# ushasigh/srsran-edgeric-5g

Measured on AMD Instinct MI355X. Metric: pdsch_slots_per_sec, higher is better.
Workload: dtype u32 bit-packed GF(2) + bf16 grid + f32 IQ

## Files before the change

### srsran-edgeric-5g_amd/csrc/bits_device.h

```cpp
#pragma once

#include "nrphy_internal.h"

namespace nrphy {

constexpr int WAVE = 64;

#ifdef NRPHY_WG_TRACE
constexpr uint32_t WG_TRACE_MAX = 16384;
__device__ uint64_t g_wg_trace[8 * WG_TRACE_MAX];
#define NRPHY_WG_TRACE_MARK(slot)                                              \
  do {                                                                         \
    if (threadIdx.x == 0 && blockIdx.x < WG_TRACE_MAX) {                       \
      g_wg_trace[8 * blockIdx.x + (slot)] = wall_clock64();                    \
    }                                                                          \
  } while (0)
#define NRPHY_WG_TRACE_WHERE(role)                                                                              \
  do {                                                                                                          \
    if (threadIdx.x == 0 && blockIdx.x < WG_TRACE_MAX) {                                                        \
      const uint64_t hw = (uint32_t)__builtin_amdgcn_s_getreg((31 << 11) | 4), xcc = (uint32_t)__builtin_amdgcn_s_getreg((31 << 11) | 20); \
      g_wg_trace[8 * blockIdx.x + 7] = ((uint64_t)(role) << 60) | ((xcc & 0xFu) << 32) | hw;                     \
    }                                                                                                           \
  } while (0)
#else
// ... 169 lines not shown
}

__device__ __forceinline__ uint32_t byte_masks_msb_first(uint32_t bits4)
{
  const uint32_t spread = ((bits4 >> 3) & 1u) | (((bits4 >> 2) & 1u) << 8) | (((bits4 >> 1) & 1u) << 16) | ((bits4 & 1u) << 24);
  return spread * 0xFFu;
}

__device__ __forceinline__ uint32_t negate_bytes(uint32_t x, uint32_t m)
{
  const uint32_t a = x ^ m, b = m & 0x01010101u;
  return ((a & 0x7F7F7F7Fu) + b) ^ (a & 0x80808080u);
}

__device__ __forceinline__ uint32_t gold_matvec(const uint32_t* rows, uint32_t state, uint32_t lane)
{
  uint32_t bit = (lane < 31u) ? (__popc(rows[lane & 31u] & state) & 1u) : 0u;
  return (uint32_t)__ballot(bit != 0) & 0x7FFFFFFFu;
}

__device__ __forceinline__ void wave_lds_fence()
{
  asm volatile("s_waitcnt lgkmcnt(0)" ::: "memory");
}

__device__ inline void gold_sequence_wave(const GoldTables* gold, const uint32_t* x1_words, uint32_t c_init,
                                          uint32_t nwords, uint32_t* __restrict__ out, uint32_t* scratch,
                                          uint32_t lane)
{
  uint32_t state = c_init & 0x7FFFFFFFu;
  state = gold_matvec(gold->x2_jump[6], state, lane);
  state = gold_matvec(gold->x2_jump[9], state, lane);
  state = gold_matvec(gold->x2_jump[10], state, lane);
  if (lane < 31u && lane < nwords) {
    uint32_t word = 0;
#pragma unroll 8
    for (uint32_t t = 0; t != 32; ++t) {
      word |= (__popc(gold->x2_head[t][lane] & state) & 1u) << (31u - t);
    }
    scratch[lane] = word;
  }
  wave_lds_fence();
  for (uint32_t base = 31; base < nwords; base += 28) {
    const uint32_t k = base + lane;
    if (lane < 28u && k < nwords) {
      scratch[k] = scratch[k - 28] ^ scratch[k - 29] ^ scratch[k - 30] ^ scratch[k - 31];
    }
    wave_lds_fence();
  }
  for (uint32_t k = lane; k < nwords; k += WAVE) {
    out[k] = scratch[k] ^ x1_words[k];
  }
}

#ifndef NRPHY_GOLD_LEVEL
#define NRPHY_GOLD_LEVEL 64
#endif
constexpr uint32_t GOLD_MAX_LEVEL  = NRPHY_GOLD_LEVEL;
constexpr uint32_t GOLD_RING_WORDS = 64 * GOLD_MAX_LEVEL;

__device__ __forceinline__ void lds_barrier()
{
  asm volatile("s_waitcnt lgkmcnt(0)\n\ts_barrier" ::: "memory");
}

template <uint32_t NT, bool WITH_X1 = true>
__device__ inline void gold_sequence_workgroup(const GoldTables* gold, const uint32_t* x1_words, uint32_t c_init,
                                               uint32_t first_word, uint32_t nwords, uint32_t* __restrict__ out,
                                               uint32_t* ring, uint32_t tid)
{
  constexpr uint32_t MASK = GOLD_RING_WORDS - 1;
  constexpr uint32_t PER  = (28u * GOLD_MAX_LEVEL + NT - 1u) / NT;
  const uint32_t     lane = tid & (WAVE - 1);
  if (nwords == 0) {
    return;
  }
  static_assert(NT == 4 * WAVE, "four waves share the seed words");
  if (tid < 31u) {
    ring[tid] = 0u;
  }
  if (tid < WAVE) {
    uint32_t       state  = c_init & 0x7FFFFFFFu;
    const uint32_t offset = 1600u + 32u * first_word;
    uint32_t row[GOLD_JUMP_BITS];
#pragma unroll
    for (uint32_t k = 0; k != GOLD_JUMP_BITS; ++k) {
      row[k] = ((offset >> k) & 1u) ? gold->x2_jump[k][lane & 31u] : 0u;
    }
#pragma unroll
    for (uint32_t k = 0; k != GOLD_JUMP_BITS; ++k) {
      if ((offset >> k) & 1u) {
        const uint32_t bit = (lane < 31u) ? (__popc(row[k] & state) & 1u) : 0u;
        state              = (uint32_t)__ballot(bit != 0) & 0x7FFFFFFFu;
      }
    }
    if (lane == 0) {
      ring[GOLD_RING_WORDS - 1u] = state;
    }
  }
  lds_barrier();
  {
    const uint32_t state = ring[GOLD_RING_WORDS - 1u];
    const uint32_t t0    = 8u * (tid / WAVE);
    if (lane < 31u) {
      uint32_t head[8];
#pragma unroll
      for (uint32_t t = 0; t != 8; ++t) {
        head[t] = gold->x2_head[t0 + t][lane];
      }
      uint32_t word = 0;
#pragma unroll
      for (uint32_t t = 0; t != 8; ++t) {
        word |= (__popc(head[t] & state) & 1u) << (31u - (t0 + t));
      }
      atomicOr(&ring[lane], word);
    }
  }
  lds_barrier();
  uint32_t pw[PER], px[PER];
  uint32_t pbeg = 0, pend = nwords < 31u ? nwords : 31u;
#pragma unroll
  for (uint32_t i = 0; i != PER; ++i) {
    const uint32_t k = tid + i * NT;
    pw[i]            = (k < pend) ? ring[k] : 0u;
    px[i]            = (WITH_X1 && k < pend) ? x1_words[first_word + k] : 0u;
  }
  uint32_t m = 1, have = 31;
  auto step = [&](uint32_t (&nw)[PER], uint32_t (&nx)[PER], const uint32_t (&ow)[PER], const uint32_t (&ox)[PER]) {
    while (m < GOLD_MAX_LEVEL && have >= 62u * m) {
      m *= 2u;
    }
    const uint32_t end = have + 28u * m < nwords ? have + 28u * m : nwords;
#pragma unroll
    for (uint32_t i = 0; i != PER; ++i) {
      const uint32_t k = have + tid + i * NT;
      nx[i]            = (WITH_X1 && k < end) ? x1_words[first_word + k] : 0u;
    }
#pragma unroll
    for (uint32_t i = 0; i != PER; ++i) {
      const uint32_t k = have + tid + i * NT;
      nw[i]            = 0;
      if (k < end) {
        nw[i] = ring[(k - 28u * m) & MASK] ^ ring[(k - 29u * m) & MASK] ^ ring[(k - 30u * m) & MASK] ^
                ring[(k - 31u * m) & MASK];
        ring[k & MASK] = nw[i];
      }
    }
#pragma unroll
    for (uint32_t i = 0; i != PER; ++i) {
      const uint32_t k = pbeg + tid + i * NT;
      if (k < pend) {
        out[k] = ow[i] ^ ox[i];
      }
    }
    pbeg = have;
    pend = end;
    lds_barrier();
    have = end;
  };
  uint32_t qw[PER], qx[PER];
  bool     in_q = false;
  while (have < nwords) {
    step(qw, qx, pw, px);
    in_q = true;
    if (have >= nwords) {
      break;
    }
    step(pw, px, qw, qx);
    in_q = false;
  }
#pragma unroll
  for (uint32_t i = 0; i != PER; ++i) {
    const uint32_t k = pbeg + tid + i * NT;
    if (k < pend) {
      out[k] = in_q ? (qw[i] ^ qx[i]) : (pw[i] ^ px[i]);
    }
  }
  lds_barrier();
}

constexpr uint32_t GOLD_SEED_ROWS  = 31;
constexpr uint32_t GOLD_SEED_WORDS = GOLD_SEED_ROWS * WAVE;

template <class OnBlock>
__device__ inline void gold_sequence_blocks_wave(const GoldTables* gold, uint32_t c_init, uint32_t first_word, uint32_t nwords,
                                                 uint32_t* area, uint32_t lane, OnBlock&& on_block)
{
  if (nwords == 0) {
    return;
  }
  uint32_t state = c_init & 0x7FFFFFFFu;
  {
    const uint32_t offset = 1600u + 32u * first_word;
    uint32_t       row[GOLD_JUMP_BITS];
#pragma unroll
    for (uint32_t k = 0; k != GOLD_JUMP_BITS; ++k) {
      row[k] = ((offset >> k) & 1u) ? gold->x2_jump[k][lane & 31u] : 0u;
    }
#pragma unroll
    for (uint32_t k = 0; k != GOLD_JUMP_BITS; ++k) {
      if ((offset >> k) & 1u) {
        const uint32_t bit = (lane < 31u) ? (__popc(row[k] & state) & 1u) : 0u;
        state              = (uint32_t)__ballot(bit != 0) & 0x7FFFFFFFu;
      }
    }
  }
  NRPHY_WG_TRACE_MARK(1);
  if (lane < 31u) {
    uint32_t head[32];
#pragma unroll
    for (uint32_t t = 0; t != 32; ++t) {
      head[t] = gold->x2_head[t][lane];
    }
    uint32_t word = 0;
#pragma unroll
    for (uint32_t t = 0; t != 32; ++t) {
      word |= (__popc(head[t] & state) & 1u) << (31u - t);
    }
    area[lane] = word;
  }
  wave_lds_fence();
  NRPHY_WG_TRACE_MARK(2);
  const uint32_t need = nwords < GOLD_SEED_WORDS ? nwords : GOLD_SEED_WORDS;
  for (uint32_t have = 31u, m = 1u; have < need;) {
    while (m < 32u && have >= 62u * m) {
      m *= 2u;
    }
    const uint32_t end = have + 28u * m < need ? have + 28u * m : need;
    for (uint32_t k = have + lane; k < end; k += WAVE) {
      area[k] = __builtin_amdgcn_bitop3_b32(area[k - 28u * m], area[k - 29u * m], area[k - 30u * m], 0x96) ^
                area[k - 31u * m];
    }
    wave_lds_fence();
    have = end;
  }
  NRPHY_WG_TRACE_MARK(3);
  on_block(0u, need);
  NRPHY_WG_TRACE_MARK(4);
  const uint32_t rows = (nwords + WAVE - 1u) / WAVE;
  if (rows <= GOLD_SEED_ROWS) {
    return;
  }
  uint32_t w[GOLD_SEED_ROWS];
#pragma unroll
  for (uint32_t i = 0; i != GOLD_SEED_ROWS; ++i) {
    w[i] = area[i * WAVE + lane];
  }
  for (uint32_t base = GOLD_SEED_ROWS; base < rows; base += GOLD_SEED_ROWS) {
#pragma unroll
    for (uint32_t i = 0; i != GOLD_SEED_ROWS; ++i) {
      w[i] ^= __builtin_amdgcn_bitop3_b32(w[(i + 1u) % GOLD_SEED_ROWS], w[(i + 2u) % GOLD_SEED_ROWS],
                                          w[(i + 3u) % GOLD_SEED_ROWS], 0x96);
      area[i * WAVE + lane] = w[i];
    }
    wave_lds_fence();
    const uint32_t left = nwords - base * WAVE;
    on_block(base * WAVE, left < GOLD_SEED_WORDS ? left : GOLD_SEED_WORDS);
  }
}

constexpr uint32_t GOLD_EXPAND_MAX_WORDS = 703;

template <uint32_t M>
__device__ __forceinline__ uint32_t gold_expand_step(uint32_t* x2, uint32_t have, uint32_t need, uint32_t lane)
{
  if (have >= need) {
    return have;
  }
  const uint32_t end = have + 28u * M < need ? have + 28u * M : need;
#pragma unroll
  for (uint32_t s = 0; s != (28u * M + WAVE - 1u) / WAVE; ++s) {
    if (have + WAVE * s >= end) {
      break;
    }
    const uint32_t k = have + lane + WAVE * s;
    if (k < end) {
      uint32_t* b = x2 + (k - 31u * M);
      b[31u * M]  = __builtin_amdgcn_bitop3_b32(b[3u * M], b[2u * M], b[M], 0x96) ^ b[0];
    }
  }
  wave_lds_fence();
  return end;
}

__device__ inline void gold_expand_seed_wave(uint32_t* x2, uint32_t seed_word, uint32_t need, uint32_t lane)
{
  if (lane < 31u) {
    x2[lane] = seed_word;
  }
  wave_lds_fence();
  uint32_t have = 31u;
  have = gold_expand_step<1>(x2, have, need, lane);
  have = gold_expand_step<1>(x2, have, need, lane);
  have = gold_expand_step<2>(x2, have, need, lane);
  have = gold_expand_step<4>(x2, have, need, lane);
  have = gold_expand_step<8>(x2, have, need, lane);
  have = gold_expand_step<8>(x2, have, need, lane);
}

constexpr int TB_CRC_THREADS = 256;

constexpr int TB_CRC_WPT = NRPHY_CRC_WORDS_PER_THREAD;
static_assert(TB_CRC_REGION_WORDS == TB_CRC_WPT * TB_CRC_THREADS, "words per thread");

__device__ __forceinline__ uint32_t crc_advance(const uint32_t* tab, uint32_t reg)
{
  return tab[reg & 0xFFu] ^ tab[256u + ((reg >> 8) & 0xFFu)] ^ tab[512u + ((reg >> 16) & 0xFFu)] ^ tab[768u + (reg >> 24)];
}

constexpr uint32_t TB_CRC_LDS_WORDS = 4 * 1024 + 2 * TB_CRC_THREADS;

__device__ inline uint32_t tbcrc_regions_workgroup(const TbCrcTables* tables, uint32_t sel, CrcPoly c, const uint32_t* tbw, uint32_t n,
                                                   uint32_t region0, uint32_t count, uint32_t factor, uint32_t* lds, uint32_t tid)
{
  uint32_t*       y32 = lds;
  uint32_t*       y1k = lds + 1024;
  uint32_t*       y8k = lds + 2048;
  uint32_t*       yz  = lds + 3072;
  uint32_t*       msg = lds + 4096;

  constexpr int   ROUNDS = TB_CRC_WPT / 4;
  static_assert(TB_CRC_WPT == 16, "the tables assume four rounds of four words (y1k, y8k)");
  const uint32_t  nwords  = (n + 3u) >> 2;
  const bool      aligned = (reinterpret_cast<uintptr_t>(tbw) & 15u) == 0;
  auto load_region = [&](uint32_t region, uint32_t (&w)[TB_CRC_WPT]) {
#pragma unroll
    for (int i = 0; i != ROUNDS; ++i) {
      const uint32_t idx = region * TB_CRC_REGION_WORDS + ((uint32_t)i * TB_CRC_THREADS + tid) * 4u;
      if (aligned && idx + 4u <= nwords && !((n & 3u) != 0 && idx + 4u == nwords)) {
        const uint4 v = *reinterpret_cast<const uint4*>(tbw + idx);
        w[4 * i] = __builtin_bswap32(v.x), w[4 * i + 1] = __builtin_bswap32(v.y);
        w[4 * i + 2] = __builtin_bswap32(v.z), w[4 * i + 3] = __builtin_bswap32(v.w);
      } else {
#pragma unroll
        for (int k = 0; k != 4; ++k) {
          uint32_t x = (idx + k < nwords) ? be_word(tbw, idx + k) : 0u;
          if ((n & 3u) != 0 && idx + k + 1u == nwords) {
            x &= 0xFFFFFFFFu << (8u * (4u - (n & 3u)));
          }
          w[4 * i + k] = x;
        }
      }
    }
  };
  uint32_t w[TB_CRC_WPT], wn[TB_CRC_WPT];
  load_region(region0, w);
#pragma unroll
  for (int k = 0; k != 4; ++k) {
    y32[k * 256 + tid] = tables->y32[sel][k][tid];
    y1k[k * 256 + tid] = tables->y1k[sel][k][tid];
    y8k[k * 256 + tid] = tables->y8k[sel][k][tid];
    yz[k * 256 + tid]  = tables->yz[sel][k][tid];
  }
  __syncthreads();
#ifdef NRPHY_WG_TRACE
  asm volatile("s_waitcnt vmcnt(0)" ::: "memory");
  NRPHY_WG_TRACE_MARK(2);
#endif
  uint32_t acc = 0;
  for (uint32_t j = 0; j != count; ++j) {
    if (j + 1u != count) {
      load_region(region0 + j + 1u, wn);
    }
    uint32_t v[ROUNDS];
#pragma unroll
    for (int i = 0; i != ROUNDS; ++i) {
      v[i] = w[4 * i];
    }
#pragma unroll
    for (int k = 1; k != 4; ++k) {
#pragma unroll
      for (int i = 0; i != ROUNDS; ++i) {
        v[i] = crc_advance(y32, v[i]) ^ w[4 * i + k];
      }
    }
    uint32_t reg = v[0];
#pragma unroll
    for (int i = 1; i != ROUNDS; ++i) {
      reg = crc_advance(y1k, reg) ^ v[i];
    }
    uint32_t* m = msg + (j & 1u) * TB_CRC_THREADS;
    m[tid]      = reg;
    lds_barrier();
    if (tid < WAVE) {
      uint32_t r = m[tid];
#pragma unroll
      for (int k = 1; k != 4; ++k) {
        r = crc_advance(y8k, r) ^ m[tid + WAVE * k];
      }
      acc = (j != 0 ? crc_advance(yz, acc) : 0u) ^ r;
    }
    if (j + 1u != count) {
#pragma unroll
      for (int i = 0; i != TB_CRC_WPT; ++i) {
        w[i] = wn[i];
      }
    }
  }
  NRPHY_WG_TRACE_MARK(1);
  uint32_t share = 0;
  if (tid < WAVE) {
    uint32_t r = crc_mulmod32(tables->lane[sel][tid], acc, c);
    r          = wave_xor(r);
    share      = crc_mulmod(r, factor, c);
  }
  return share;
}

__device__ __forceinline__ uint32_t to_bf16_bits(float v)
{
  uint32_t u = __float_as_uint(v);
  u += 0x7FFFu + ((u >> 16) & 1u);
  return u >> 16;
}

__device__ __forceinline__ float2 cbf16_to_float2(uint32_t w)
{
  return make_float2(__uint_as_float(w << 16), __uint_as_float(w & 0xFFFF0000u));
}

__device__ __forceinline__ double wave_sum(double x)
{
#pragma unroll
  for (int o = WAVE / 2; o != 0; o >>= 1) {
    x += __shfl_xor(x, o);
  }
  return x;
}

}
```

### srsran-edgeric-5g_amd/csrc/pdsch_kernels.hip

```cpp
#include "ldpc_device.h"

#ifndef NRPHY_PHASE_A_STAGED
#define NRPHY_PHASE_A_STAGED 1
#endif

#ifdef NRPHY_PROBES
#define NRPHY_STAGE(p) ((p).profile_stage)
#else
#define NRPHY_STAGE(p) 0u
#endif

namespace nrphy {

__global__ __launch_bounds__(TB_CRC_THREADS) void prologue_kernel(PdschLaunch p, const uint8_t* __restrict__ d_tb)
{
  constexpr uint32_t LDS_WORDS = TB_CRC_LDS_WORDS;
  __shared__ __attribute__((aligned(16))) uint32_t lds[LDS_WORDS];
  static_assert(LDS_WORDS >= GOLD_RING_WORDS, "LDS of the sequence role");
  const uint32_t tid = threadIdx.x;

  uint32_t scr_index = blockIdx.x, crc_index = blockIdx.x - p.n_scr_work;
  bool     scr_role  = blockIdx.x < p.n_scr_work;
  if (p.prologue_order == 1 && p.n_scr_work != 0 && p.n_crc_work != 0) {
    const uint32_t total = p.n_scr_work + p.n_crc_work;
    const uint32_t xcd = blockIdx.x & 7u, turn = blockIdx.x >> 3, q = total >> 3, r = total & 7u;
    const uint32_t pos = xcd * q + (xcd < r ? xcd : r) + turn;
    const uint32_t s0 = (uint32_t)(((uint64_t)pos * p.n_scr_work + total - 1u) / total);
    const uint32_t s1 = (uint32_t)(((uint64_t)(pos + 1u) * p.n_scr_work + total - 1u) / total);
    scr_role  = s1 > s0;
    scr_index = s0;
    crc_index = pos - s0;
  }
  NRPHY_WG_TRACE_MARK(0);
  NRPHY_WG_TRACE_WHERE(scr_role ? 1 : 2);
  if (scr_role) {
    if (NRPHY_STAGE(p) == 8) {
      return;
    }
    const auto*    swc   = to_constant(&p.scr_work[scr_index]);
    const uint32_t first = swc->first, count = swc->count;
    const bool     with_dmrs = swc->with_dmrs != 0;
    PduRef         pd    = *to_constant(&p.pdus[swc->pdu]);
    const uint32_t wave = tid / WAVE, lane = tid % WAVE;
    constexpr uint32_t DMRS_WAVES = TB_CRC_THREADS / WAVE - 1, DMRS_SCRATCH = (GOLD_RING_WORDS - 2048u) / DMRS_WAVES;
    static_assert(GOLD_SEED_WORDS <= 2048u && GOLD_RING_WORDS > 2048u, "LDS of the sequence role");
    static_assert((12u * NRPHY_MAX_RB + 31u) / 32u + 1u <= DMRS_SCRATCH, "DM-RS scratch per wave");
    if (wave == 0) {
      if (count == 0) {
        return;
      }
      const uint32_t lq = pd.qm * pd.nof_layers, n_short = pd.n_short, e_short = pd.e_short, e_long = pd.e_long, C = pd.C;
      const uint32_t nre_short = e_short / lq, nre_long = e_long / lq;
      struct Cursor {
        uint32_t cb, re_begin, item, bit_cb, nre;
      };
      Cursor resume = {0u, 0u, pd.seed_first, 0u, n_short != 0 ? nre_short : nre_long};
      auto   advance = [&](Cursor& c) {
        c.re_begin += RE_CHUNK;
        if (c.re_begin >= c.nre) {
          c.bit_cb += c.cb < n_short ? e_short : e_long;
          ++c.cb;
          c.re_begin = 0;
          c.nre      = c.cb < n_short ? nre_short : nre_long;
        }
        ++c.item;
      };
      gold_sequence_blocks_wave(p.gold, pd.c_init, first, count, lds, lane, [&](uint32_t base, uint32_t avail) {
        const uint32_t lo = first + base, hi = lo + avail;
        Cursor c        = resume;
        bool   resuming = false;
        while (c.cb < C) {
          const uint32_t w0 = (c.bit_cb + c.re_begin * lq) >> 5;
          if (w0 >= hi) {
            break;
          }
          if (w0 + 31u > lo) {
            const uint32_t k = w0 + lane;
            if (lane < 31u && k >= lo && k < hi) {
              p.scr_seed[(size_t)c.item * 32u + lane] = lds[k - lo];
            }
          }
          if (w0 + 31u > hi && !resuming) {
            resume   = c;
            resuming = true;
          }
          advance(c);
        }
        if (!resuming) {
          resume = c;
        }
      });
      NRPHY_WG_TRACE_MARK(6);
    } else if (with_dmrs && pd.dmrs_seq_words <= DMRS_SCRATCH) {
      uint32_t ordinal = 0;
      for (uint32_t mask = pd.dmrs_symbol_mask; mask != 0; mask &= mask - 1u, ++ordinal) {
        if (ordinal % DMRS_WAVES == wave - 1u) {
          const uint32_t l = (uint32_t)__ffs(mask) - 1u;
          gold_sequence_wave(p.gold, p.x1_words, pd.dmrs_c_init[l], pd.dmrs_seq_words,
                             p.scr + pd.dmrs_seq_offset + ordinal * pd.dmrs_seq_words,
                             lds + 2048u + (wave - 1u) * DMRS_SCRATCH, lane);
        }
      }
    }
    return;
  }

  if (NRPHY_STAGE(p) == 9) {
    return;
  }
  const auto*     wkc = to_constant(&p.crc_work[crc_index]);
  const uint32_t  wk_pdu = wkc->pdu, wk_region = wkc->region, wk_factor = wkc->factor, wk_count = wkc->count;
  PduRef          pd  = *to_constant(&p.pdus[wk_pdu]);
  const uint32_t  sel = (pd.tb_crc_bits == 16) ? 1u : 0u;
  const CrcPoly   c   = sel ? crc16() : crc24a();
  const uint32_t  n   = pd.tb_bytes;
  const uint32_t* tbw = reinterpret_cast<const uint32_t*>(d_tb + pd.tb_offset);
#ifdef NRPHY_WG_TRACE
  asm volatile("s_waitcnt lgkmcnt(0)" ::: "memory");
  NRPHY_WG_TRACE_MARK(3);
#endif
  const uint32_t share = tbcrc_regions_workgroup(p.tbcrc, sel, c, tbw, n, wk_region, wk_count, wk_factor, lds, tid);
  if (tid == 0) {
    p.tb_crc_part[crc_index] = share;
  }
  NRPHY_WG_TRACE_MARK(6);
}

#ifdef NRPHY_WG_TRACE
extern "C" int nrphy_debug_wg_trace(uint64_t* out, uint32_t nof_blocks)
{
  const size_t n = 8 * (size_t)(nof_blocks < WG_TRACE_MAX ? nof_blocks : WG_TRACE_MAX) * sizeof(uint64_t);
  return (int)hipMemcpyFromSymbol(out, HIP_SYMBOL(g_wg_trace), n, 0, hipMemcpyDeviceToHost);
}
#endif

hipError_t launch_prologue(const PdschLaunch& p, const uint8_t* d_tb, hipStream_t stream)
{
  if (p.n_crc_work + p.n_scr_work == 0) {
    return hipSuccess;
  }
  hipLaunchKernelGGL(prologue_kernel, dim3(p.n_crc_work + p.n_scr_work), dim3(TB_CRC_THREADS), 0, stream, p, d_tb);
  return hipGetLastError();
}

constexpr uint32_t CB_U_QAM_WORDS     = 512;
constexpr uint32_t CB_U_LDPC_WORDS    = (sizeof(LdpcScratch) / 4u + 3u) & ~3u;
constexpr uint32_t CB_U_GRAPH_OFFSET  = LDPC_DBL_WORDS + CB_U_LDPC_WORDS;
static_assert(CB_U_GRAPH_OFFSET == NRPHY_CB_U_GRAPH_OFFSET, "host and device agree on the layout of the scratch region");

struct CbShared {
  uint32_t* lin;
  uint32_t* u;
  uint32_t* symb;
  uint32_t* graph;
  LdpcScratch* ldpc;
};

#ifndef NRPHY_LDS_PROBE
#define NRPHY_LDS_PROBE 0
#endif
__device__ __forceinline__ uint32_t lds_probe_index(uint32_t idx, uint32_t bit)
{
  if ((NRPHY_LDS_PROBE >> bit) & 1) {
    uint32_t zero = 0;
    asm volatile("" : "+v"(zero));
    const uint32_t lane = __builtin_amdgcn_mbcnt_hi(~0u, __builtin_amdgcn_mbcnt_lo(~0u, 0u));
    return (idx & zero) + lane;
  }
  return idx;
}

__device__ __forceinline__ uint32_t crc24_word_step(const uint32_t* tab, uint32_t reg, uint32_t word)
{
#if NRPHY_CRC_SLICES == 4
  const uint32_t v = (reg << 8) ^ word;
  return tab[v & 0xFFu] ^ tab[256u + ((v >> 8) & 0xFFu)] ^ tab[512u + ((v >> 16) & 0xFFu)] ^ tab[768u + (v >> 24)];
#else
  const uint32_t v = reg ^ (word >> 8);
  uint32_t       r = tab[lds_probe_index(v & 0xFFu, 1)] ^ tab[256u + lds_probe_index((v >> 8) & 0xFFu, 1)] ^ tab[512u + lds_probe_index(v >> 16, 1)];
  return ((r << 8) & 0xFFFFFFu) ^ tab[lds_probe_index(((r >> 16) ^ word) & 0xFFu, 1)];
#endif
}

__device__ inline void build_codeblock(PduRef pd, uint32_t cb, const uint32_t* tbw, const uint32_t* tb_crc_part,
                                       const GoldTables* tables, CbShared* sh, uint32_t total_words, uint32_t lane,
                                       uint32_t profile_stage)
{
  const bool     last    = (cb == pd.C - 1);
  const uint32_t used    = pd.info_bits - (last ? pd.tb_crc_bits + pd.zero_pad : 0u);
  const uint32_t tb_pos  = cb * pd.info_bits;
  const uint32_t tb_bits = pd.tb_bytes * 8u;
  const uint4* crc_src = reinterpret_cast<const uint4*>(&tables->crc24b_slice[0][0]);
  const uint4  crc_tab0 = crc_src[lane], crc_tab1 = crc_src[lane + WAVE], crc_tab2 = crc_src[lane + 2 * WAVE];
#if NRPHY_CRC_SLICES == 4
  const uint4 crc_tab3 = crc_src[lane + 3 * WAVE];
#endif
  constexpr uint32_t SEG_UNROLL = 5;
  for (uint32_t base = lane; base < total_words; base += WAVE * SEG_UNROLL) {
    uint32_t hi[SEG_UNROLL], lo[SEG_UNROLL];
#pragma unroll
    for (uint32_t k = 0; k != SEG_UNROLL; ++k) {
      const uint32_t pos = 32u * (base + WAVE * k);
      hi[k] = 0;
      lo[k] = 0;
      if (pos < used) {
        const uint32_t abs_pos = tb_pos + pos;
        const uint32_t i = abs_pos >> 5, sft = abs_pos & 31u;
        hi[k] = tbw[i];
        if (sft != 0 && 32u * (i + 1) < tb_bits) {
          lo[k] = tbw[i + 1];
        }
      }
    }
#pragma unroll
    for (uint32_t k = 0; k != SEG_UNROLL; ++k) {
      const uint32_t j = base + WAVE * k, pos = 32u * j;
      if (j < total_words) {
        uint32_t v = 0;
        if (pos < used) {
          v = __funnelshift_l(__builtin_bswap32(lo[k]), __builtin_bswap32(hi[k]), (tb_pos + pos) & 31u);
          const uint32_t remaining = used - pos;
          if (remaining < 32u) {
            v &= topmask(remaining);
          }
        }
        sh->lin[j] = v;
      }
    }
  }
  {
    uint4* dst           = reinterpret_cast<uint4*>(sh->u);
    dst[lane]            = crc_tab0;
    dst[lane + WAVE]     = crc_tab1;
    dst[lane + 2 * WAVE] = crc_tab2;
#if NRPHY_CRC_SLICES == 4
    dst[lane + 3 * WAVE] = crc_tab3;
#endif
  }
  wave_sync();
  if (profile_stage == 7) {
    return;
  }
  if (last) {
    const uint32_t tb_crc = wave_xor(lane < pd.crc_count ? tb_crc_part[pd.crc_first + lane] : 0u);
    if (lane == 0) {
      or_bits_lds_exclusive(sh->lin, used, tb_crc << (32u - pd.tb_crc_bits), pd.tb_crc_bits);
    }
  }
  wave_sync();
  if (pd.cb_crc_bits) {
    const uint32_t n   = pd.info_bits;
    const uint32_t pad = (32u - (n & 31u)) & 31u;
    const uint32_t nw  = (n + pad) >> 5;
    const uint32_t per = (nw + WAVE - 1) / WAVE;
    uint32_t       a   = lane * per;
    uint32_t       b   = a + per;
    a                  = a > nw ? nw : a;
    b                  = b > nw ? nw : b;
    uint32_t reg       = 0;
    for (uint32_t j = a; j < b; ++j) {
      uint32_t word;
      if (pad == 0) {
        word = sh->lin[j];
      } else if (j == 0) {
        word = sh->lin[0] >> pad;
      } else {
        word = ext32(sh->lin, 32u * j - pad);
      }
      reg = crc24_word_step(sh->u, reg, word);
    }
    uint32_t part = 0;
    {
      const uint32_t m = nw - b;
#pragma unroll
      for (uint32_t k = 0; k != 6; ++k) {
        part ^= tables->crc24b_mul[m][k][(reg >> (4u * k)) & 15u];
      }
    }
    uint32_t crc = wave_xor(part);
    if (lane == 0) {
      or_bits_lds_exclusive(sh->lin, n, crc << 8, 24);
    }
    wave_sync();
  }
}

struct RmIndex {
  uint32_t fs;
  uint32_t flen;
  uint32_t n_valid;
  uint32_t rank0;
  float    inv_valid;
};

__device__ __forceinline__ RmIndex rm_index_init(PduRef pd)
{
  RmIndex  r;
  uint32_t nsys = (pd.kb - 2u) * pd.zc;
  uint32_t fs   = nsys - pd.filler;
  uint32_t fe   = nsys;
  fs            = fs > pd.n_cb ? pd.n_cb : fs;
  fe            = fe > pd.n_cb ? pd.n_cb : fe;
  r.fs          = fs;
  r.flen        = fe - fs;
  r.n_valid     = pd.n_cb - r.flen;
  r.rank0       = pd.k0 < fs ? pd.k0 : (pd.k0 < fe ? fs : pd.k0 - r.flen);
  r.inv_valid   = 1.0f / (float)r.n_valid;
  return r;
}

template <bool WRAP>
__device__ __forceinline__ uint32_t rm_gather32(const RmIndex& r, const uint32_t* lin, uint32_t zc2, uint32_t t)
{
  uint32_t u = r.rank0 + t;
  if (WRAP && u >= r.n_valid) {
    uint32_t q = (uint32_t)((float)u * r.inv_valid);
    u -= q * r.n_valid;
    if ((int32_t)u < 0) {
      u += r.n_valid;
    } else if (u >= r.n_valid) {
      u -= r.n_valid;
    }
  }
  uint32_t run = (u < r.fs) ? r.fs - u : r.n_valid - u;
  uint32_t out = ext32(lin, (u < r.fs ? u : u + r.flen) + zc2);
  if (run >= 32u) {
    return out;
  }
  out &= topmask(run);
  uint32_t filled = run;
  while (filled < 32u) {
    u += run;
    if (u >= r.n_valid) {
      if (!WRAP) {
        break;
      }
      u = 0;
    }
    run            = (u < r.fs) ? r.fs - u : r.n_valid - u;
    run            = run > 32u - filled ? 32u - filled : run;
    uint32_t piece = ext32(lin, (u < r.fs ? u : u + r.flen) + zc2);
    out |= (piece & topmask(run)) >> filled;
    filled += run;
  }
  return out;
}

__device__ __forceinline__ uint32_t bit_select(uint32_t m, uint32_t a, uint32_t b)
{
  return __builtin_amdgcn_bitop3_b32(m, a, b, 0xCA);
}

__device__ __forceinline__ void transpose8x8(uint32_t& hi, uint32_t& lo)
{
  hi = bit_select(0xAA55AA55u, hi, bit_select(0x55005500u, hi << 7, hi >> 7));
  lo = bit_select(0xAA55AA55u, lo, bit_select(0x55005500u, lo << 7, lo >> 7));
  hi = bit_select(0xCCCC3333u, hi, bit_select(0x33330000u, hi << 14, hi >> 14));
  lo = bit_select(0xCCCC3333u, lo, bit_select(0x33330000u, lo << 14, lo >> 14));
  const uint32_t nhi = bit_select(0xF0F0F0F0u, hi, lo >> 4);
  const uint32_t nlo = bit_select(0x0F0F0F0Fu, lo, hi << 4);
  hi                 = nhi;
  lo                 = nlo;
}

__device__ __forceinline__ void cmul_ref(float xr, float xi, float wr, float wi, float& outr, float& outi)
{
  float t0 = __fmul_rn(xi, wi);
  float t1 = __fmul_rn(xr, wi);
  outr     = __fmaf_rn(xr, wr, -t0);
  outi     = __fmaf_rn(xi, wr, t1);
}

typedef float cf2 __attribute__((ext_vector_type(2)));
__device__ __forceinline__ cf2 cmul_ref_packed(cf2 x, cf2 w)
{
  cf2 t, r;
  asm("v_pk_mul_f32 %0, %1, %2 op_sel:[1,1] op_sel_hi:[0,1]" : "=v"(t) : "v"(x), "v"(w));
  asm("v_pk_fma_f32 %0, %1, %2, %3 op_sel_hi:[1,0,1] neg_lo:[0,0,1]" : "=v"(r) : "v"(x), "v"(w), "v"(t));
  return r;
}
__device__ __forceinline__ cf2 cmul_ref_packed_uniform(cf2 x, cf2 w)
{
  cf2 t, r;
  asm("v_pk_mul_f32 %0, %1, %2 op_sel:[1,1] op_sel_hi:[0,1]" : "=v"(t) : "v"(x), "s"(w));
  asm("v_pk_fma_f32 %0, %1, %2, %3 op_sel_hi:[1,0,1] neg_lo:[0,0,1]" : "=v"(r) : "v"(x), "s"(w), "v"(t));
  return r;
}

typedef __bf16 bf16x2_t __attribute__((ext_vector_type(2)));
typedef float  f32x2_t __attribute__((ext_vector_type(2)));
__device__ __forceinline__ uint32_t pack_cbf16(float re, float im)
{
  f32x2_t  v = {re, im};
  bf16x2_t b = __builtin_convertvector(v, bf16x2_t);
  return *reinterpret_cast<uint32_t*>(&b);
}

__device__ __forceinline__ void grid_store(uint32_t* p, uint32_t v)
{
  __builtin_nontemporal_store(v, p);
}

#ifndef NRPHY_GRID_STORE_AUX
#define NRPHY_GRID_STORE_AUX 2
#endif
#ifndef NRPHY_GRID_BUFFER_STORES
#define NRPHY_GRID_BUFFER_STORES 1
#endif

struct ChunkGeom {
  uint32_t E;
  uint32_t cw_cb;
  uint32_t bit0;
};

template <int QM, int L, bool WRAP>
__device__ __forceinline__ void phase_a(const PdschLaunch& p, PduRef pd, const CbWork& wk, const CbShared& sh,
                                        uint32_t E, uint32_t lane)
{
  const uint32_t esym = E / QM;
  const uint32_t zc2  = 2u * pd.zc;
  const RmIndex  rm   = rm_index_init(pd);
  const uint32_t s0   = wk.re_begin * L;
  const uint32_t nblk = (wk.re_count * L + 31u) >> 5;
  constexpr uint32_t LUT_TRIPS = ((1u << QM) + WAVE - 1u) / WAVE;
  float2             lut[LUT_TRIPS];
#pragma unroll
  for (uint32_t k = 0; k != LUT_TRIPS; ++k) {
    lut[k] = lane + WAVE * k < (1u << QM) ? p.gold->qam_lut[QM / 2 - 1][lane + WAVE * k] : make_float2(0.f, 0.f);
  }
#if NRPHY_PHASE_A_STAGED
  for (uint32_t item = lane; item < QM * nblk; item += WAVE) {
    const uint32_t blk = item / QM, j = item - blk * QM;
    sh.symb[8u * blk + j] = rm_gather32<WRAP>(rm, sh.lin, zc2, j * esym + s0 + 32u * blk);
  }
  wave_sync();
  const uint8_t* rows = reinterpret_cast<const uint8_t*>(sh.symb);
  for (uint32_t item = lane; item < 4u * nblk; item += WAVE) {
    const uint32_t blk = item >> 2, m = item & 3u;
    const uint8_t* b   = rows + 32u * blk + (3u - m);
    uint32_t       r8[8];
#pragma unroll
    for (int j = 0; j != 8; ++j) {
      r8[j] = (j < QM) ? b[4 * j] : 0u;
    }
    uint32_t hi = (r8[0] << 24) | (r8[1] << 16) | (r8[2] << 8) | r8[3];
    uint32_t lo = (r8[4] << 24) | (r8[5] << 16) | (r8[6] << 8) | r8[7];
    transpose8x8(hi, lo);
    sh.symb[8u * blk + 2u * m]      = hi;
    sh.symb[8u * blk + 2u * m + 1u] = lo;
  }
#else
  for (uint32_t blk = lane; blk < nblk; blk += WAVE) {
    uint32_t row[8];
#pragma unroll
    for (int j = 0; j != 8; ++j) {
      row[j] = (j < QM) ? rm_gather32<WRAP>(rm, sh.lin, zc2, (uint32_t)j * esym + s0 + 32u * blk) : 0u;
    }
#pragma unroll
    for (int m = 0; m != 4; ++m) {
      const int sft = 24 - 8 * m;
      uint32_t  hi  = (((row[0] >> sft) & 0xFFu) << 24) | (((row[1] >> sft) & 0xFFu) << 16) |
                    (((row[2] >> sft) & 0xFFu) << 8) | ((row[3] >> sft) & 0xFFu);
      uint32_t lo = (((row[4] >> sft) & 0xFFu) << 24) | (((row[5] >> sft) & 0xFFu) << 16) |
                    (((row[6] >> sft) & 0xFFu) << 8) | ((row[7] >> sft) & 0xFFu);
      transpose8x8(hi, lo);
      sh.symb[8u * blk + 2u * m]      = hi;
      sh.symb[8u * blk + 2u * m + 1u] = lo;
    }
  }
#endif
  if (lane < 8) {
    sh.symb[8u * nblk + lane] = 0;
  }
// ... 742 lines not shown
```

Measured before the change: 1.291 million.

## Give each wave its own TB CRC chunk and drop per-region workgroup barrier

The transport-block CRC loop now assigns each wave a contiguous chunk of every region and keeps a per-wave running accumulator. This removes the LDS exchange and barrier that the old code ran on every region iteration. The per-wave results are combined once at the end with the y1k table before the lane-weight multiply, which reassigns the roles of the y1k and y8k tables. Byte-swapping moves from the load to the reduce step, loads are guarded per chunk, and the LDS message buffer is halved. The risk is correctness of the reassigned combine tables and more scalar work in the tail path.

```diff
diff --git a/srsran-edgeric-5g_amd/csrc/bits_device.h b/srsran-edgeric-5g_amd/csrc/bits_device.h
--- a/srsran-edgeric-5g_amd/csrc/bits_device.h
+++ b/srsran-edgeric-5g_amd/csrc/bits_device.h
@@ -495,13 +495,29 @@
 
 constexpr int TB_CRC_WPT = NRPHY_CRC_WORDS_PER_THREAD;
 static_assert(TB_CRC_REGION_WORDS == TB_CRC_WPT * TB_CRC_THREADS, "words per thread");
+constexpr uint32_t TB_CRC_CHUNK_WORDS = TB_CRC_WPT * WAVE;
+
+#ifndef NRPHY_LDS_PROBE
+#define NRPHY_LDS_PROBE 0
+#endif
+__device__ __forceinline__ uint32_t lds_probe_index(uint32_t idx, uint32_t bit)
+{
+  if ((NRPHY_LDS_PROBE >> bit) & 1) {
+    uint32_t zero = 0;
+    asm volatile("" : "+v"(zero));
+    const uint32_t lane = __builtin_amdgcn_mbcnt_hi(~0u, __builtin_amdgcn_mbcnt_lo(~0u, 0u));
+    return (idx & zero) + lane;
+  }
+  return idx;
+}
 
 __device__ __forceinline__ uint32_t crc_advance(const uint32_t* tab, uint32_t reg)
 {
-  return tab[reg & 0xFFu] ^ tab[256u + ((reg >> 8) & 0xFFu)] ^ tab[512u + ((reg >> 16) & 0xFFu)] ^ tab[768u + (reg >> 24)];
-}
-
-constexpr uint32_t TB_CRC_LDS_WORDS = 4 * 1024 + 2 * TB_CRC_THREADS;
+  return tab[lds_probe_index(reg & 0xFFu, 2)] ^ tab[256u + lds_probe_index((reg >> 8) & 0xFFu, 2)] ^
+         tab[512u + lds_probe_index((reg >> 16) & 0xFFu, 2)] ^ tab[768u + lds_probe_index(reg >> 24, 2)];
+}
+
+constexpr uint32_t TB_CRC_LDS_WORDS = 4 * 1024 + TB_CRC_THREADS;
 
 __device__ inline uint32_t tbcrc_regions_workgroup(const TbCrcTables* tables, uint32_t sel, CrcPoly c, const uint32_t* tbw, uint32_t n,
                                                    uint32_t region0, uint32_t count, uint32_t factor, uint32_t* lds, uint32_t tid)
@@ -511,33 +527,37 @@
   uint32_t*       y8k = lds + 2048;
   uint32_t*       yz  = lds + 3072;
   uint32_t*       msg = lds + 4096;
+  const uint32_t  wave = (uint32_t)__builtin_amdgcn_readfirstlane((int)(tid / WAVE)), lane = tid % WAVE;
 
   constexpr int   ROUNDS = TB_CRC_WPT / 4;
-  static_assert(TB_CRC_WPT == 16, "the tables assume four rounds of four words (y1k, y8k)");
-  const uint32_t  nwords  = (n + 3u) >> 2;
+  static_assert(TB_CRC_WPT == 16 && TB_CRC_THREADS == 4 * WAVE, "the tables assume four waves, four rounds of four words (y1k, y8k)");
+  const uint32_t  nwords  = (n + 3u) >> 2, nfull = n >> 2;
   const bool      aligned = (reinterpret_cast<uintptr_t>(tbw) & 15u) == 0;
-  auto load_region = [&](uint32_t region, uint32_t (&w)[TB_CRC_WPT]) {
-#pragma unroll
-    for (int i = 0; i != ROUNDS; ++i) {
-      const uint32_t idx = region * TB_CRC_REGION_WORDS + ((uint32_t)i * TB_CRC_THREADS + tid) * 4u;
-      if (aligned && idx + 4u <= nwords && !((n & 3u) != 0 && idx + 4u == nwords)) {
-        const uint4 v = *reinterpret_cast<const uint4*>(tbw + idx);
-        w[4 * i] = __builtin_bswap32(v.x), w[4 * i + 1] = __builtin_bswap32(v.y);
-        w[4 * i + 2] = __builtin_bswap32(v.z), w[4 * i + 3] = __builtin_bswap32(v.w);
-      } else {
-#pragma unroll
-        for (int k = 0; k != 4; ++k) {
-          uint32_t x = (idx + k < nwords) ? be_word(tbw, idx + k) : 0u;
-          if ((n & 3u) != 0 && idx + k + 1u == nwords) {
-            x &= 0xFFFFFFFFu << (8u * (4u - (n & 3u)));
-          }
-          w[4 * i + k] = x;
-        }
+  auto chunk_base = [&](uint32_t region) { return region * TB_CRC_REGION_WORDS + wave * TB_CRC_CHUNK_WORDS; };
+  auto load_chunk = [&](uint32_t region, uint32_t (&w)[TB_CRC_WPT]) {
+    const uint32_t base = chunk_base(region);
+    if (base >= nwords) {
+      return;
+    }
+    if (aligned && base + TB_CRC_CHUNK_WORDS <= nfull) {
+#pragma unroll
+      for (int i = 0; i != ROUNDS; ++i) {
+        const uint4 v = *reinterpret_cast<const uint4*>(tbw + base + ((uint32_t)i * WAVE + lane) * 4u);
+        w[4 * i] = v.x, w[4 * i + 1] = v.y, w[4 * i + 2] = v.z, w[4 * i + 3] = v.w;
+      }
+    } else {
+      const uint32_t tail_mask = (n & 3u) != 0 ? 0xFFFFFFFFu >> (8u * (4u - (n & 3u))) : 0xFFFFFFFFu;
+#pragma unroll
+      for (int i = 0; i != TB_CRC_WPT; ++i) {
+        const uint32_t idx = base + ((uint32_t)(i / 4) * WAVE + lane) * 4u + (uint32_t)(i % 4);
+        const uint32_t keep = idx + 1u < nwords ? 0xFFFFFFFFu : idx + 1u == nwords ? tail_mask : 0u;
+        w[i] = tbw[idx < nwords ? idx : nwords - 1u] & keep;
       }
     }
   };
-  uint32_t w[TB_CRC_WPT], wn[TB_CRC_WPT];
-  load_region(region0, w);
+  uint32_t w[TB_CRC_WPT] = {}, wn[TB_CRC_WPT] = {};
+  load_chunk(region0, w);
+  const uint32_t lane_weight = tables->lane[sel][lane];
 #pragma unroll
   for (int k = 0; k != 4; ++k) {
     y32[k * 256 + tid] = tables->y32[sel][k][tid];
@@ -551,38 +571,34 @@
   NRPHY_WG_TRACE_MARK(2);
 #endif
   uint32_t acc = 0;
+  auto reduce_chunk = [&](uint32_t j, const uint32_t (&x)[TB_CRC_WPT]) {
+    uint32_t reg = 0;
+    if (chunk_base(region0 + j) < nwords) {
+      uint32_t v[ROUNDS];
+#pragma unroll
+      for (int i = 0; i != ROUNDS; ++i) {
+        v[i] = __builtin_bswap32(x[4 * i]);
+      }
+#pragma unroll
+      for (int k = 1; k != 4; ++k) {
+#pragma unroll
+        for (int i = 0; i != ROUNDS; ++i) {
+          v[i] = crc_advance(y32, v[i]) ^ __builtin_bswap32(x[4 * i + k]);
+        }
+      }
+      reg = v[0];
+#pragma unroll
+      for (int i = 1; i != ROUNDS; ++i) {
+        reg = crc_advance(y8k, reg) ^ v[i];
+      }
+    }
+    acc = (j != 0 ? crc_advance(yz, acc) : 0u) ^ reg;
+  };
   for (uint32_t j = 0; j != count; ++j) {
     if (j + 1u != count) {
-      load_region(region0 + j + 1u, wn);
-    }
-    uint32_t v[ROUNDS];
-#pragma unroll
-    for (int i = 0; i != ROUNDS; ++i) {
-      v[i] = w[4 * i];
-    }
-#pragma unroll
-    for (int k = 1; k != 4; ++k) {
-#pragma unroll
-      for (int i = 0; i != ROUNDS; ++i) {
-        v[i] = crc_advance(y32, v[i]) ^ w[4 * i + k];
-      }
-    }
-    uint32_t reg = v[0];
-#pragma unroll
-    for (int i = 1; i != ROUNDS; ++i) {
-      reg = crc_advance(y1k, reg) ^ v[i];
-    }
-    uint32_t* m = msg + (j & 1u) * TB_CRC_THREADS;
-    m[tid]      = reg;
-    lds_barrier();
-    if (tid < WAVE) {
-      uint32_t r = m[tid];
-#pragma unroll
-      for (int k = 1; k != 4; ++k) {
-        r = crc_advance(y8k, r) ^ m[tid + WAVE * k];
-      }
-      acc = (j != 0 ? crc_advance(yz, acc) : 0u) ^ r;
-    }
+      load_chunk(region0 + j + 1u, wn);
+    }
+    reduce_chunk(j, w);
     if (j + 1u != count) {
 #pragma unroll
       for (int i = 0; i != TB_CRC_WPT; ++i) {
@@ -591,11 +607,18 @@
     }
   }
   NRPHY_WG_TRACE_MARK(1);
+  msg[tid] = acc;
+  __syncthreads();
   uint32_t share = 0;
   if (tid < WAVE) {
-    uint32_t r = crc_mulmod32(tables->lane[sel][tid], acc, c);
-    r          = wave_xor(r);
-    share      = crc_mulmod(r, factor, c);
+    uint32_t r = msg[tid];
+#pragma unroll
+    for (int k = 1; k != 4; ++k) {
+      r = crc_advance(y1k, r) ^ msg[tid + WAVE * k];
+    }
+    r     = crc_mulmod32(lane_weight, r, c);
+    r     = wave_xor(r);
+    share = crc_mulmod(r, factor, c);
   }
   return share;
 }
diff --git a/srsran-edgeric-5g_amd/csrc/pdsch_kernels.hip b/srsran-edgeric-5g_amd/csrc/pdsch_kernels.hip
--- a/srsran-edgeric-5g_amd/csrc/pdsch_kernels.hip
+++ b/srsran-edgeric-5g_amd/csrc/pdsch_kernels.hip
@@ -156,20 +156,6 @@
   LdpcScratch* ldpc;
 };
 
-#ifndef NRPHY_LDS_PROBE
-#define NRPHY_LDS_PROBE 0
-#endif
-__device__ __forceinline__ uint32_t lds_probe_index(uint32_t idx, uint32_t bit)
-{
-  if ((NRPHY_LDS_PROBE >> bit) & 1) {
-    uint32_t zero = 0;
-    asm volatile("" : "+v"(zero));
-    const uint32_t lane = __builtin_amdgcn_mbcnt_hi(~0u, __builtin_amdgcn_mbcnt_lo(~0u, 0u));
-    return (idx & zero) + lane;
-  }
-  return idx;
-}
-
 __device__ __forceinline__ uint32_t crc24_word_step(const uint32_t* tab, uint32_t reg, uint32_t word)
 {
 #if NRPHY_CRC_SLICES == 4
```

Result: no change. 1.300 million (median of 6 runs) (+0.7%).
